# Napoliee/Expressive-FastSpeech2-Mandarin

Hardware: AMD Instinct MI355X
Metric: mel-frames/sec/GPU (batch-64 synth) at 1/2/4/8 MI355X; RTF (higher is better)
Workload: dtype bf16; 1 GPU; cfg2: batch=64 x 64 phonemes per GPU, ESD-Chinese-Singing-MFA model.yaml, FastSpeech2.forward eval bf16; global_batch=64, seq_len=64, mel_frames_per_gpu_batch=24883, T_max=430, parallelism=dp1 (independent shards, no collective), hip_graph=True

## Files before the change

expressive-fastspeech2-mandarin_amd/csrc/ffn_wide.hip:

```cpp
#include <cstdlib>
#include <type_traits>
#include <utility>

#include "conv_common.h"
#include "fs2_common.h"

#ifndef WIDE_TRACE
#define WIDE_TRACE 0
#endif

namespace {

constexpr int kWD = 256;
constexpr int kWUnit = 4096;
constexpr int kWLgkm0 = 0xC07F;

template <int N, typename Fn, int... I>
__device__ __forceinline__ void wfor_impl(Fn &&f, std::integer_sequence<int, I...>) {
  (f(std::integral_constant<int, I>{}), ...);
}
template <int N, typename Fn>
__device__ __forceinline__ void wfor(Fn &&f) {
  wfor_impl<N>(f, std::make_integer_sequence<int, N>{});
}

struct WideArgs {
  const bf16 *x;
  int64_t xs;
  uint32_t x_bytes;
  const bf16 *w;
  uint32_t w_bytes;
  const float *b1, *b2, *gamma, *beta;
  float eps;
  const int64_t *lens;
  const float *av1, *av2;
  const int *rows_dev;
  const int2 *row_pos;
  int M, T, pad, F;
  bf16 *h;
  uint32_t h_bytes;
  int *cnt;
  float *z;
  uint32_t z_bytes;
  bf16 *out;
  int64_t os;
  int nslices, ntiles;
  uint64_t *trace;
};

struct Stamps {
  uint64_t t[8];
  int n = 0;
  __device__ __forceinline__ void at() {
    if (WIDE_TRACE) {
      __builtin_amdgcn_sched_barrier(0);
      t[n++] = __builtin_readcyclecounter();
      __builtin_amdgcn_sched_barrier(0);
    }
  }
  __device__ __forceinline__ void put(uint64_t *tr, int slot) {
    if (WIDE_TRACE && tr != nullptr && threadIdx.x == 0 && slot < 512) {
      for (int i = 0; i < n; ++i) tr[slot * 8 + i] = t[i];
      tr[slot * 8 + 7] = (uint64_t)n;
    }
  }
};

template <int KS>
__global__ __launch_bounds__(256, 2) void ffn_hidden_kernel(WideArgs p) {
  constexpr int BM = 256, XROWS = BM + KS - 1;
  constexpr int NPC = (XROWS + 15) / 16;
  constexpr int CH = 64 + NPC * 1024;
  constexpr int NCH = kWD / 32;
  constexpr int PPW = (NPC + 3) / 4;
  constexpr int NSLOT = 3;
  constexpr int SMEM = NSLOT * CH;
  static_assert(2 * SMEM <= 163840, "two workgroups per CU");
  static_assert(BM * 144 <= SMEM, "H staging fits in the ring");
  static_assert((NSLOT - 1) * CH < 65536, "slot offsets fit the ds_read immediate");
  constexpr int NK = KS * NCH;
  constexpr int MB = 8;
  __shared__ __attribute__((aligned(16))) char smem[SMEM];
  Stamps st;
  st.at();

  const int tid = threadIdx.x, lane = tid & 63;
  const int w = __builtin_amdgcn_readfirstlane(tid >> 6);
  const int rh = w & 1, hh = w >> 1;
  const int L = (blockIdx.x & 7) * (gridDim.x >> 3) + (blockIdx.x >> 3);
  const int slice = L / p.ntiles, tile = L - slice * p.ntiles;
  if (slice >= p.nslices) return;
  const int M = p.rows_dev != nullptr ? min(*p.rows_dev, p.M) : p.M;
  const int m0 = tile * BM;
  if (m0 >= M) return;
  const int pad = p.pad, T = p.T;

  if (tid < NSLOT * 4) *reinterpret_cast<float4 *>(smem + (tid >> 2) * CH + (tid & 3) * 16) = make_float4(0.f, 0.f, 0.f, 0.f);
  int2 rq[MB];
#pragma unroll
  for (int mb = 0; mb < MB; ++mb) {
    const int m = min(m0 + rh * 128 + mb * 16 + (lane & 15), M - 1);
    rq[mb] = make_int2(m % T, T);
  }
  if (p.row_pos != nullptr) {
#pragma unroll
    for (int mb = 0; mb < MB; ++mb) rq[mb] = p.row_pos[min(m0 + rh * 128 + mb * 16 + (lane & 15), M - 1)];
  }
  const int hcol0 = slice * 64 + hh * 32 + 4 * (lane >> 4);
  const float4 bb0 = *reinterpret_cast<const float4 *>(p.b1 + hcol0);
  const float4 bb1 = *reinterpret_cast<const float4 *>(p.b1 + hcol0 + 16);
  const rsrc_t sr = make_rsrc(p.x, p.x_bytes);
  const uint32_t srow = (uint32_t)p.xs * 2u;
  auto dma_chunk = [&](auto CI) {
    constexpr int c = decltype(CI)::value;
    const int ps = lane & 3;
#pragma unroll
    for (int i = 0; i < PPW; ++i) {
      const int pc = min(w + 4 * i, NPC - 1);
      const int R = pc * 16 + (lane >> 2);
      const int hl = ps ^ ((R >> 1) & 2);
      const int gm = m0 - pad + R;
      const bool ok = R < XROWS && gm >= 0 && gm < M;
      __builtin_amdgcn_raw_ptr_buffer_load_lds(
          sr, (__attribute__((address_space(3))) void *)(smem + (c % NSLOT) * CH + 64 + pc * 1024), 16,
          ok ? (uint32_t)gm * srow + (uint32_t)(c * 64 + hl * 16) : kOOB, 0, 0, 0);
    }
  };
  dma_chunk(std::integral_constant<int, 0>{});
  dma_chunk(std::integral_constant<int, 1>{});

  constexpr int RD = 6;
  const rsrc_t wr = make_rsrc(p.w, p.w_bytes);
  const uint32_t wbase = (uint32_t)(slice * NK) * (uint32_t)kWUnit + (uint32_t)(hh * 2048 + lane * 16);
  bf16x8 pa[RD][2];
  auto load_at = [&](auto KI) {
    constexpr int kk = decltype(KI)::value, c = kk / KS, t = kk % KS;
    __builtin_amdgcn_sched_barrier(0);
    const uint32_t o = wbase + (uint32_t)(t * NCH + c) * (uint32_t)kWUnit;
    pa[kk % RD][0] = __builtin_bit_cast(bf16x8, __builtin_amdgcn_raw_buffer_load_b128(wr, o, 0, 0));
    pa[kk % RD][1] = __builtin_bit_cast(bf16x8, __builtin_amdgcn_raw_buffer_load_b128(wr, o + 1024, 0, 0));
    __builtin_amdgcn_sched_barrier(0);
  };
  wfor<RD>([&](auto I) { load_at(I); });
  auto refills = [](int a, int b) constexpr {
    int n = 0;
    for (int kk = a; kk <= b; ++kk) n += kk + RD < NK ? 2 : 0;
    return n;
  };

  const int r16 = lane & 15, hi = lane >> 4;
  uint32_t adp[KS][MB / 2];
  {
    asm volatile("s_waitcnt vmcnt(%0)" ::"n"(2 * PPW + 2 * RD) : "memory");
#pragma unroll
    for (int t = 0; t < KS; ++t) {
      const int R0 = rh * 128 + r16 + t;
      const int sl = (hi ^ ((R0 >> 1) & 2)) * 16;
#pragma unroll
      for (int i = 0; i < MB / 2; ++i) {
        uint32_t a2[2];
#pragma unroll
        for (int j = 0; j < 2; ++j) {
          const int mb = 2 * i + j;
          const bool ok = (unsigned)(rq[mb].x + t - pad) < (unsigned)rq[mb].y;
          a2[j] = ok ? (uint32_t)(64 + (R0 + 16 * mb) * 64 + sl) : 0u;
        }
        adp[t][i] = a2[0] | (a2[1] << 16);
      }
    }
  }
  static_assert(CH < 65536, "16-bit fragment addresses");
  auto wait_chunk = [&](auto CI) {
    constexpr int c = decltype(CI)::value;
    constexpr int n = c == 0 ? PPW + 2 * RD
                             : c == 1 ? 2 * RD + refills(0, KS - 2)
                                      : refills((c - 2) * KS + KS - 1, (c - 1) * KS + KS - 2);
    static_assert(n <= 63, "vmcnt");
    asm volatile("s_waitcnt vmcnt(%0)" ::"n"(n) : "memory");
    __builtin_amdgcn_s_waitcnt(kWLgkm0);
    __builtin_amdgcn_sched_barrier(0);
    __builtin_amdgcn_s_barrier();
    __builtin_amdgcn_sched_barrier(0);
  };
  wait_chunk(std::integral_constant<int, 0>{});
  st.at();

  f32x4 acc[2][MB];
#pragma unroll
  for (int jb = 0; jb < 2; ++jb)
#pragma unroll
    for (int mb = 0; mb < MB; ++mb) acc[jb][mb] = f32x4{0.f, 0.f, 0.f, 0.f};
  auto issue = [&](auto CI, auto TI, bf16x8 (&f)[MB]) {
    constexpr int c = decltype(CI)::value, t = decltype(TI)::value, off = (c % NSLOT) * CH;
#pragma unroll
    for (int mb = 0; mb < MB; ++mb) {
      uint32_t a;
      asm volatile("v_bfe_u32 %0, %1, %2, 16" : "=v"(a) : "v"(adp[t][mb >> 1]), "n"((mb & 1) * 16));
      f[mb] = *reinterpret_cast<const bf16x8 *>(smem + a + off);
    }
  };
  auto mma = [&](const bf16x8 (&fa)[2], const bf16x8 (&fb)[MB]) {
#pragma unroll
    for (int mb = 0; mb < MB; ++mb)
#pragma unroll
      for (int jb = 0; jb < 2; ++jb)
        acc[jb][mb] = __builtin_amdgcn_mfma_f32_16x16x32_bf16(fa[jb], fb[mb], acc[jb][mb], 0, 0, 0);
  };
  bf16x8 f0[MB], f1[MB];
  issue(std::integral_constant<int, 0>{}, std::integral_constant<int, 0>{}, f0);
  wfor<NCH>([&](auto CI) {
    constexpr int c = decltype(CI)::value;
    wfor<KS>([&](auto TI) {
      constexpr int t = decltype(TI)::value;
      constexpr int kk = c * KS + t;
      if constexpr (t + 1 < KS) {
        if constexpr (kk & 1)
          issue(CI, std::integral_constant<int, t + 1>{}, f0);
        else
          issue(CI, std::integral_constant<int, t + 1>{}, f1);
      } else if constexpr (c + 1 < NCH) {
        wait_chunk(std::integral_constant<int, c + 1>{});
        if constexpr (c + 2 < NCH) dma_chunk(std::integral_constant<int, c + 2>{});
        if constexpr (kk & 1)
          issue(std::integral_constant<int, c + 1>{}, std::integral_constant<int, 0>{}, f0);
        else
          issue(std::integral_constant<int, c + 1>{}, std::integral_constant<int, 0>{}, f1);
      }
      if constexpr (kk & 1)
        mma(pa[kk % RD], f1);
      else
        mma(pa[kk % RD], f0);
      if constexpr (kk + RD < NK) load_at(std::integral_constant<int, kk + RD>{});
    });
  });
  __builtin_amdgcn_s_waitcnt(kWLgkm0);
  __builtin_amdgcn_s_barrier();
  st.at();

  constexpr int HP = 144;
  const int hrow0 = rh * 128 + r16;
#pragma unroll
  for (int jb = 0; jb < 2; ++jb) {
    const float4 bb = jb == 0 ? bb0 : bb1;
#pragma unroll
    for (int mb = 0; mb < MB; ++mb) {
      const f32x4 v = acc[jb][mb];
      bf16x4 o;
      o[0] = (bf16)fmaxf(v[0] + bb.x, 0.f);
      o[1] = (bf16)fmaxf(v[1] + bb.y, 0.f);
      o[2] = (bf16)fmaxf(v[2] + bb.z, 0.f);
      o[3] = (bf16)fmaxf(v[3] + bb.w, 0.f);
      *reinterpret_cast<bf16x4 *>(smem + (hrow0 + 16 * mb) * HP + (hh * 32 + jb * 16 + 4 * hi) * 2) = o;
    }
  }
  __builtin_amdgcn_s_waitcnt(kWLgkm0);
  __syncthreads();
  const uint32_t hrow = (uint32_t)p.F * 2u;
  char *hb = reinterpret_cast<char *>(p.h);
#pragma unroll
  for (int i = 0; i < BM * 8 / 256; ++i) {
    const int e = tid + 256 * i, r = e >> 3, c = e & 7;
    if (m0 + r < M)
      *reinterpret_cast<uint4 *>(hb + (uint32_t)(m0 + r) * hrow + (uint32_t)(slice * 128 + c * 16)) =
          *reinterpret_cast<const uint4 *>(smem + r * HP + c * 16);
  }
  if (WIDE_TRACE) {
    asm volatile("s_waitcnt vmcnt(0)" ::: "memory");
    st.at();
    st.put(p.trace, L);
  }
}

__device__ __forceinline__ void ln_row(const WideArgs &p, f32x4 (&v)[16], int m, int hi, const char *vec, char *dst) {
  bool masked = false;
  int bb = 0;
  if (p.row_pos == nullptr) {
    bb = m / p.T;
    masked = p.lens != nullptr && (int64_t)(m - bb * p.T) >= p.lens[bb];
  }
  float4 a1[16], a2[16];
#pragma unroll
  for (int i = 0; i < 16; ++i) {
    const int n = 16 * i + 4 * hi;
    a1[i] = p.av1 != nullptr ? *reinterpret_cast<const float4 *>(p.av1 + (int64_t)bb * kWD + n) : make_float4(0.f, 0.f, 0.f, 0.f);
  }
  float s = 0.f;
#pragma unroll
  for (int i = 0; i < 16; ++i) s += (v[i][0] + v[i][1]) + (v[i][2] + v[i][3]);
  s += __shfl_xor(s, 16, 64);
  s += __shfl_xor(s, 32, 64);
  const float mean = s * (1.0f / 256.0f);
  float ss = 0.f;
#pragma unroll
  for (int i = 0; i < 16; ++i) {
    v[i] -= mean;
    ss += (v[i][0] * v[i][0] + v[i][1] * v[i][1]) + (v[i][2] * v[i][2] + v[i][3] * v[i][3]);
  }
  ss += __shfl_xor(ss, 16, 64);
  ss += __shfl_xor(ss, 32, 64);
  const float rstd = 1.0f / sqrtf(ss * (1.0f / 256.0f) + p.eps);
#pragma unroll
  for (int i = 0; i < 16; ++i) {
    const int n = 16 * i + 4 * hi;
    a2[i] = p.av2 != nullptr ? *reinterpret_cast<const float4 *>(p.av2 + (int64_t)bb * kWD + n) : make_float4(0.f, 0.f, 0.f, 0.f);
  }
  const float *vg = reinterpret_cast<const float *>(vec), *vb = vg + kWD;
#pragma unroll
  for (int i = 0; i < 16; ++i) {
    const int n = 16 * i + 4 * hi;
    const float4 g = *reinterpret_cast<const float4 *>(vg + n);
    const float4 be = *reinterpret_cast<const float4 *>(vb + n);
    float y[4] = {v[i][0] * rstd * g.x + be.x, v[i][1] * rstd * g.y + be.y, v[i][2] * rstd * g.z + be.z,
                  v[i][3] * rstd * g.w + be.w};
    if (masked) y[0] = y[1] = y[2] = y[3] = 0.f;
    if (p.av1 != nullptr) {
      y[0] += a1[i].x; y[1] += a1[i].y; y[2] += a1[i].z; y[3] += a1[i].w;
    }
    if (p.av2 != nullptr) {
      y[0] += a2[i].x; y[1] += a2[i].y; y[2] += a2[i].z; y[3] += a2[i].w;
    }
    const bf16x4 o = {(bf16)y[0], (bf16)y[1], (bf16)y[2], (bf16)y[3]};
    *reinterpret_cast<bf16x4 *>(dst + n * 2) = o;
  }
}

template <int F, int RB>
__global__ __launch_bounds__(256, 1) void ffn_out_rows_kernel(WideArgs p) {
  constexpr int NK = F / 32;
  constexpr int KW = NK / 4;
  constexpr int BM = 16 * RB;
  constexpr int RD = 3;
  static_assert(KW >= RD && (RD - 1) * (16 + RB) <= 63, "ring");
  constexpr int RED = 4 * 16 * RB * 64 * 16;
  constexpr int ZP = kWD * 4 + 64;
  constexpr int ZB = BM * ZP;
  constexpr int OP = kWD * 2 + 16;
  constexpr int VEC = RED;
  static_assert(ZB + BM * OP <= RED, "pre-norm rows + staging fit over the partials");
  static_assert(RED + 2048 <= 163840, "LDS");
  __shared__ __attribute__((aligned(16))) char smem[RED + 2048];
  Stamps st;
  st.at();

  const int tid = threadIdx.x, lane = tid & 63;
  const int w = __builtin_amdgcn_readfirstlane(tid >> 6);
  const int L = (blockIdx.x & 7) * (gridDim.x >> 3) + (blockIdx.x >> 3);
  if (L >= p.ntiles) return;
  const int M = p.rows_dev != nullptr ? min(*p.rows_dev, p.M) : p.M;
  const int m0 = L * BM;
  if (m0 >= M) return;
  const int hi = lane >> 4, r16 = lane & 15;
  if (w < 2)
    __builtin_amdgcn_raw_ptr_buffer_load_lds(make_rsrc(w == 0 ? p.gamma : p.beta, 1024),
                                             (__attribute__((address_space(3))) void *)(smem + VEC + w * 1024), 16,
                                             (uint32_t)lane * 16u, 0, 0, 0);
  const rsrc_t xr = make_rsrc(p.x, p.x_bytes);
  float4 b2v[4];
  uint2 xv[RB][4];
#pragma unroll
  for (int jb = 0; jb < 4; ++jb) {
    const int n = 64 * w + 16 * jb + 4 * hi;
    b2v[jb] = *reinterpret_cast<const float4 *>(p.b2 + n);
#pragma unroll
    for (int mb = 0; mb < RB; ++mb) {
      const int m = m0 + 16 * mb + r16;
      xv[mb][jb] = bload8(xr, m < M ? (uint32_t)m * (uint32_t)p.xs * 2u + (uint32_t)n * 2u : kOOB);
    }
  }

  const rsrc_t wr = make_rsrc(p.w, p.w_bytes);
  const rsrc_t hr = make_rsrc(p.h, p.h_bytes);
  const uint32_t wb = p.w_bytes - (uint32_t)(kWD * F * 2) + (uint32_t)(w * KW * kWUnit) + (uint32_t)lane * 16u;
  const uint32_t hrow = (uint32_t)F * 2u;
  uint32_t hoff[RB];
#pragma unroll
  for (int mb = 0; mb < RB; ++mb) {
    const int m = m0 + 16 * mb + r16;
    hoff[mb] = m < M ? (uint32_t)m * hrow + (uint32_t)(w * KW * 64 + hi * 16) : kOOB;
  }
  bf16x8 wa[RD][16], hb[RD][RB];
  auto load_at = [&](auto KI) {
    constexpr int k = decltype(KI)::value;
    __builtin_amdgcn_sched_barrier(0);
#pragma unroll
    for (int J = 0; J < 16; ++J)
      wa[k % RD][J] = __builtin_bit_cast(
          bf16x8, __builtin_amdgcn_raw_buffer_load_b128(wr, wb + (uint32_t)(((J >> 2) * NK + k) * kWUnit + (J & 3) * 1024), 0, 0));
#pragma unroll
    for (int mb = 0; mb < RB; ++mb)
      hb[k % RD][mb] = __builtin_bit_cast(bf16x8, __builtin_amdgcn_raw_buffer_load_b128(hr, hoff[mb] + (uint32_t)(k * 64), 0, 0));
    __builtin_amdgcn_sched_barrier(0);
  };
  wfor<RD>([&](auto I) { load_at(I); });
  if (WIDE_TRACE) st.at();

  f32x4 acc[16][RB];
#pragma unroll
  for (int J = 0; J < 16; ++J)
#pragma unroll
    for (int mb = 0; mb < RB; ++mb) acc[J][mb] = f32x4{0.f, 0.f, 0.f, 0.f};
  wfor<KW>([&](auto KI) {
    constexpr int k = decltype(KI)::value;
#pragma unroll
    for (int mb = 0; mb < RB; ++mb)
#pragma unroll
      for (int J = 0; J < 16; ++J)
        acc[J][mb] = __builtin_amdgcn_mfma_f32_16x16x32_bf16(wa[k % RD][J], hb[k % RD][mb], acc[J][mb], 0, 0, 0);
    if constexpr (k + RD < KW) load_at(std::integral_constant<int, k + RD>{});
  });
  f32x4 *red = reinterpret_cast<f32x4 *>(smem);
#pragma unroll
  for (int J = 0; J < 16; ++J)
#pragma unroll
    for (int mb = 0; mb < RB; ++mb) red[((w * 16 + J) * RB + mb) * 64 + lane] = acc[J][mb];
  asm volatile("s_waitcnt vmcnt(0)" ::: "memory");
  __builtin_amdgcn_s_waitcnt(kWLgkm0);
  __builtin_amdgcn_s_barrier();
  st.at();
  f32x4 zv[RB][4];
#pragma unroll
  for (int mb = 0; mb < RB; ++mb)
#pragma unroll
    for (int jb = 0; jb < 4; ++jb) {
      const int J = 4 * w + jb;
      f32x4 s = red[((0 * 16 + J) * RB + mb) * 64 + lane];
#pragma unroll
      for (int ww = 1; ww < 4; ++ww) s += red[((ww * 16 + J) * RB + mb) * 64 + lane];
      const bf16x4 x4 = __builtin_bit_cast(bf16x4, xv[mb][jb]);
      s[0] = s[0] + b2v[jb].x + (float)x4[0];
      s[1] = s[1] + b2v[jb].y + (float)x4[1];
      s[2] = s[2] + b2v[jb].z + (float)x4[2];
      s[3] = s[3] + b2v[jb].w + (float)x4[3];
      zv[mb][jb] = s;
    }
  __builtin_amdgcn_s_waitcnt(kWLgkm0);
  __builtin_amdgcn_s_barrier();
#pragma unroll
  for (int mb = 0; mb < RB; ++mb)
#pragma unroll
    for (int jb = 0; jb < 4; ++jb)
      *reinterpret_cast<f32x4 *>(smem + (16 * mb + r16) * ZP + (64 * w + 16 * jb + 4 * hi) * 4) = zv[mb][jb];
  __builtin_amdgcn_s_waitcnt(kWLgkm0);
  __builtin_amdgcn_s_barrier();
  st.at();
  if (w < RB && m0 + 16 * w + r16 < M) {
    f32x4 v[16];
#pragma unroll
    for (int i = 0; i < 16; ++i) v[i] = *reinterpret_cast<const f32x4 *>(smem + (16 * w + r16) * ZP + (16 * i + 4 * hi) * 4);
    ln_row(p, v, m0 + 16 * w + r16, hi, smem + VEC, smem + ZB + (16 * w + r16) * OP);
  }
  __builtin_amdgcn_s_waitcnt(kWLgkm0);
  __builtin_amdgcn_s_barrier();
#pragma unroll
  for (int i = 0; i < BM * 32 / 256; ++i) {
    const int e = tid + 256 * i, r = e >> 5, c = e & 31;
    if (m0 + r < M)
      *reinterpret_cast<uint4 *>(p.out + (int64_t)(m0 + r) * p.os + c * 8) =
          *reinterpret_cast<const uint4 *>(smem + ZB + r * OP + c * 16);
  }
  if (WIDE_TRACE) {
    asm volatile("s_waitcnt vmcnt(0)" ::: "memory");
    st.at();
    st.put(p.trace, L);
  }
}

template <int F>
__global__ __launch_bounds__(256, 1) void ffn_out_kernel(WideArgs p) {
  constexpr int NK = F / 32;
  constexpr int KW = NK / 4;
  constexpr int RED = 4 * 16 * 64 * 16;
  constexpr int VEC = RED;
  constexpr int OP = kWD * 2 + 16;
  static_assert(64 * OP <= RED, "staging fits");
  __shared__ __attribute__((aligned(16))) char smem[RED + 2048 + 16];
  Stamps st;
  st.at();

  const int tid = threadIdx.x, lane = tid & 63;
  const int w = __builtin_amdgcn_readfirstlane(tid >> 6);
  const int L = (blockIdx.x & 7) * (gridDim.x >> 3) + (blockIdx.x >> 3);
  const int tile = L >> 2, q = L & 3;
  if (tile >= p.ntiles) return;
  const int M = p.rows_dev != nullptr ? min(*p.rows_dev, p.M) : p.M;
  const int m0 = tile * 64;
  if (m0 >= M) return;
  const int hi = lane >> 4, r16 = lane & 15;
  if (w < 2)
    __builtin_amdgcn_raw_ptr_buffer_load_lds(make_rsrc(w == 0 ? p.gamma : p.beta, 1024),
                                             (__attribute__((address_space(3))) void *)(smem + VEC + w * 1024), 16,
                                             (uint32_t)lane * 16u, 0, 0, 0);

  const rsrc_t wr = make_rsrc(p.w, p.w_bytes);
  const rsrc_t hr = make_rsrc(p.h, p.h_bytes);
  bf16x8 wa[KW][4], hb[KW][4];
  const uint32_t wb = p.w_bytes - (uint32_t)(kWD * F * 2) + (uint32_t)((q * NK + w * KW) * kWUnit) + (uint32_t)lane * 16u;
  const uint32_t hrow = (uint32_t)F * 2u;
#pragma unroll
  for (int k = 0; k < KW; ++k) {
#pragma unroll
    for (int jb = 0; jb < 4; ++jb)
      wa[k][jb] = __builtin_bit_cast(bf16x8, __builtin_amdgcn_raw_buffer_load_b128(wr, wb + k * kWUnit + jb * 1024, 0, 0));
#pragma unroll
    for (int mb = 0; mb < 4; ++mb) {
      const int m = m0 + mb * 16 + r16;
      hb[k][mb] = __builtin_bit_cast(
          bf16x8, __builtin_amdgcn_raw_buffer_load_b128(
                      hr, m < M ? (uint32_t)m * hrow + (uint32_t)((w * KW + k) * 64 + hi * 16) : kOOB, 0, 0));
    }
  }
  const int m = m0 + 16 * w + r16;
  const bool mok = m < M;
  const rsrc_t xr = make_rsrc(p.x, p.x_bytes);
  const rsrc_t zr = make_rsrc(p.z, p.z_bytes);
  float4 b2v[4];
  uint2 xv[4];
#pragma unroll
  for (int jb = 0; jb < 4; ++jb) {
    const int n = 64 * q + 16 * jb + 4 * hi;
    b2v[jb] = *reinterpret_cast<const float4 *>(p.b2 + n);
    xv[jb] = bload8(xr, mok ? (uint32_t)m * (uint32_t)p.xs * 2u + (uint32_t)n * 2u : kOOB);
  }
  __builtin_amdgcn_sched_barrier(0);
  if (WIDE_TRACE) {
    asm volatile("s_waitcnt vmcnt(0)" ::: "memory");
    st.at();
  }
  f32x4 acc[4][4];
#pragma unroll
  for (int jb = 0; jb < 4; ++jb)
#pragma unroll
    for (int mb = 0; mb < 4; ++mb) acc[jb][mb] = f32x4{0.f, 0.f, 0.f, 0.f};
#pragma unroll
  for (int k = 0; k < KW; ++k)
#pragma unroll
    for (int mb = 0; mb < 4; ++mb)
#pragma unroll
      for (int jb = 0; jb < 4; ++jb)
        acc[jb][mb] = __builtin_amdgcn_mfma_f32_16x16x32_bf16(wa[k][jb], hb[k][mb], acc[jb][mb], 0, 0, 0);
  f32x4 *red = reinterpret_cast<f32x4 *>(smem);
#pragma unroll
  for (int jb = 0; jb < 4; ++jb)
#pragma unroll
    for (int mb = 0; mb < 4; ++mb) red[(w * 16 + jb * 4 + mb) * 64 + lane] = acc[jb][mb];
  __builtin_amdgcn_s_waitcnt(kWLgkm0);
  __builtin_amdgcn_s_barrier();
  st.at();
  f32x4 zv[4];
#pragma unroll
  for (int jb = 0; jb < 4; ++jb) {
    f32x4 s = red[(0 * 16 + jb * 4 + w) * 64 + lane];
#pragma unroll
    for (int ww = 1; ww < 4; ++ww) s += red[(ww * 16 + jb * 4 + w) * 64 + lane];
    zv[jb] = s;
  }
#pragma unroll
  for (int jb = 0; jb < 4; ++jb) {
    const int n = 64 * q + 16 * jb + 4 * hi;
    const bf16x4 x4 = __builtin_bit_cast(bf16x4, xv[jb]);
    f32x4 v = zv[jb];
    v[0] = v[0] + b2v[jb].x + (float)x4[0];
    v[1] = v[1] + b2v[jb].y + (float)x4[1];
    v[2] = v[2] + b2v[jb].z + (float)x4[2];
    v[3] = v[3] + b2v[jb].w + (float)x4[3];
    __builtin_amdgcn_raw_buffer_store_b128(__builtin_bit_cast(__attribute__((ext_vector_type(4))) unsigned, v), zr,
                                           mok ? ((uint32_t)m * kWD + (uint32_t)n) * 4u : kOOB, 0, 16);
  }
  asm volatile("s_waitcnt vmcnt(0)" ::: "memory");
  __syncthreads();
  st.at();
  int *flag = reinterpret_cast<int *>(smem + RED + 2048);
  if (tid == 0) {
    const int old = __hip_atomic_fetch_add(p.cnt + tile, 1, __ATOMIC_RELAXED, __HIP_MEMORY_SCOPE_AGENT);
    const int last = old == 3;
    if (last) __hip_atomic_store(p.cnt + tile, 0, __ATOMIC_RELAXED, __HIP_MEMORY_SCOPE_AGENT);
    *flag = last;
  }
  __syncthreads();
  st.at();
  if (!*flag) {
    st.put(p.trace, L);
    return;
  }

  if (mok) {
    f32x4 v[16];
#pragma unroll
    for (int i = 0; i < 16; ++i)
      v[i] = __builtin_bit_cast(f32x4, __builtin_amdgcn_raw_buffer_load_b128(
                                           zr, ((uint32_t)m * kWD + (uint32_t)(16 * i + 4 * hi)) * 4u, 0, 16));
    ln_row(p, v, m, hi, smem + VEC, smem + (16 * w + r16) * OP);
  }
  __builtin_amdgcn_s_waitcnt(kWLgkm0);
  __builtin_amdgcn_s_barrier();
#pragma unroll
  for (int i = 0; i < 8; ++i) {
    const int e = tid + 256 * i, r = e >> 5, c = e & 31;
    if (m0 + r < M)
      *reinterpret_cast<uint4 *>(p.out + (int64_t)(m0 + r) * p.os + c * 8) =
          *reinterpret_cast<const uint4 *>(smem + r * OP + c * 16);
  }
  if (WIDE_TRACE) {
    asm volatile("s_waitcnt vmcnt(0)" ::: "memory");
    st.at();
    st.put(p.trace, L);
  }
}

}

extern "C" int fs2_ffn_wide(const fs2_ffn_desc *d, void *hidden, int64_t hidden_bytes, fs2_stream_t stream) {
  if (d == nullptr || d->x == nullptr || d->w == nullptr || d->b1 == nullptr || d->b2 == nullptr ||
      d->ln_gamma == nullptr || d->ln_beta == nullptr || d->out == nullptr || hidden == nullptr)
    return FS2_EINVAL;
  if (d->B < 0 || d->T < 0 || d->x_row_stride < kWD || (d->x_row_stride & 7) || d->out_row_stride < kWD ||
      (d->out_row_stride & 7))
    return FS2_EINVAL;
  if (d->D != kWD || !(d->F == 1024 || d->F == 512) || !(d->KS == 9 || d->KS == 3) || d->pad < 0 ||
      d->pad > d->KS - 1)
    return FS2_EUNSUPPORTED;
  if (d->wqkv != nullptr || d->pre_att != nullptr) return FS2_EUNSUPPORTED;
  if ((d->rows_dev == nullptr) != (d->row_pos == nullptr)) return FS2_EINVAL;
  if (d->rows_dev != nullptr && (d->lens != nullptr || d->addvec1 != nullptr || d->addvec2 != nullptr))
    return FS2_EINVAL;
  if (d->x == d->out || hidden == d->x || hidden == d->out) return FS2_EINVAL;
  const int64_t M64 = (int64_t)d->B * d->T;
  if (M64 > 0x7fffff00LL || d->rows_max < 0) return FS2_EINVAL;
  if (M64 == 0) return FS2_OK;
  const int64_t Mg = (d->rows_dev != nullptr && d->rows_max > 0 && d->rows_max < M64) ? d->rows_max : M64;
  const int64_t xb = M64 * d->x_row_stride * 2;
  const int64_t wb = ((int64_t)d->F * d->KS * kWD + (int64_t)kWD * d->F) * 2;
  const int64_t hb = Mg * d->F * 2;
  const int ntiles64 = (int)((Mg + 63) / 64);
  const int64_t zb = Mg * kWD * 4;
  if (xb >= (1LL << 31) || hb >= (1LL << 31) || hidden_bytes < hb) return FS2_EUNSUPPORTED;
  if (d->splitk_ws == nullptr || ntiles64 > 1024 || d->splitk_ws_bytes < 4096 + zb || zb >= (1LL << 31))
    return FS2_EINVAL;
  WideArgs p{};
  p.x = reinterpret_cast<const bf16 *>(d->x);
  p.xs = d->x_row_stride;
  p.x_bytes = (uint32_t)xb;
  p.w = reinterpret_cast<const bf16 *>(d->w);
  p.w_bytes = (uint32_t)wb;
  p.b1 = d->b1;
  p.b2 = d->b2;
  p.gamma = d->ln_gamma;
  p.beta = d->ln_beta;
  p.eps = d->ln_eps;
  p.lens = d->lens;
  p.av1 = d->addvec1;
  p.av2 = d->addvec2;
  p.rows_dev = d->rows_dev;
  p.row_pos = reinterpret_cast<const int2 *>(d->row_pos);
  p.M = (int)Mg;
  p.T = d->T;
  p.pad = d->pad;
  p.F = d->F;
  p.h = static_cast<bf16 *>(hidden);
  p.h_bytes = (uint32_t)hb;
  p.cnt = static_cast<int *>(d->splitk_ws);
  p.z = reinterpret_cast<float *>(static_cast<char *>(d->splitk_ws) + 4096);
  p.z_bytes = (uint32_t)zb;
  p.out = static_cast<bf16 *>(d->out);
  p.os = d->out_row_stride;
  if (WIDE_TRACE)
    p.trace = reinterpret_cast<uint64_t *>(static_cast<char *>(d->splitk_ws) + d->splitk_ws_bytes - 65536);
  hipStream_t s = as_stream(stream);
  p.nslices = d->F / 64;
  p.ntiles = (int)((Mg + 255) / 256);
  const int n1 = (p.nslices * p.ntiles + 7) & ~7;
  constexpr int kCUs = 256;
  constexpr int kRowsRounds = 2;
  const size_t solo = 32 * 1024;
  if (d->KS == 9)
    hipLaunchKernelGGL((ffn_hidden_kernel<9>), dim3(n1), dim3(256), n1 <= kCUs ? solo : 0, s, p);
  else
    hipLaunchKernelGGL((ffn_hidden_kernel<3>), dim3(n1), dim3(256), n1 <= kCUs ? solo : 0, s, p);
  FS2_CHECK_LAUNCH();
  if (WIDE_TRACE) p.trace += 4096;
  {
    const char *e = getenv("FS2_WIDE_OUT"), *f = getenv("FS2_WIDE_OUT_RB");
    int rb = 0;
    if (e == nullptr || e[0] != '0') {
      if (f != nullptr && (f[0] == '1' || f[0] == '2'))
        rb = f[0] - '0';
      else
        rb = Mg <= 16 * kCUs ? 1 : Mg <= 32 * kRowsRounds * kCUs ? 2 : 0;
    }
    if (rb != 0) {
      p.ntiles = (int)((Mg + 16 * rb - 1) / (16 * rb));
      const int nr = (p.ntiles + 7) & ~7;
      if (d->F == 1024 && rb == 1)
        hipLaunchKernelGGL((ffn_out_rows_kernel<1024, 1>), dim3(nr), dim3(256), 0, s, p);
      else if (d->F == 1024)
        hipLaunchKernelGGL((ffn_out_rows_kernel<1024, 2>), dim3(nr), dim3(256), 0, s, p);
      else if (rb == 1)
        hipLaunchKernelGGL((ffn_out_rows_kernel<512, 1>), dim3(nr), dim3(256), 0, s, p);
      else
        hipLaunchKernelGGL((ffn_out_rows_kernel<512, 2>), dim3(nr), dim3(256), 0, s, p);
      FS2_CHECK_LAUNCH();
      return FS2_OK;
    }
  }
  p.ntiles = ntiles64;
  const int n2 = (ntiles64 * 4 + 7) & ~7;
  if (d->F == 1024)
    hipLaunchKernelGGL((ffn_out_kernel<1024>), dim3(n2), dim3(256), 0, s, p);
  else
    hipLaunchKernelGGL((ffn_out_kernel<512>), dim3(n2), dim3(256), 0, s, p);
  FS2_CHECK_LAUNCH();
  return FS2_OK;
}
```

Baseline: 18.17 million mel-frames/s.

## Use 8-wave workgroups for FFN hidden kernel when grid underfills CUs

Templates the FFN hidden conv-GEMM kernel on wave count, so an 8-wave (512-thread) variant splits each 256-row tile into four row groups of 64 rows instead of two of 128. The 8-wave version is picked when the grid is no larger than the CU count, and an env var can force either variant. The aim is more waves per CU for latency hiding and less per-wave work in the underfilled case. In exchange it runs one workgroup per CU, and the trace also records hardware IDs.

```diff
diff --git a/expressive-fastspeech2-mandarin_amd/csrc/ffn_wide.hip b/expressive-fastspeech2-mandarin_amd/csrc/ffn_wide.hip
--- a/expressive-fastspeech2-mandarin_amd/csrc/ffn_wide.hip
+++ b/expressive-fastspeech2-mandarin_amd/csrc/ffn_wide.hip
@@ -61,32 +61,37 @@
   __device__ __forceinline__ void put(uint64_t *tr, int slot) {
     if (WIDE_TRACE && tr != nullptr && threadIdx.x == 0 && slot < 512) {
       for (int i = 0; i < n; ++i) tr[slot * 8 + i] = t[i];
+      tr[slot * 8 + 6] = (uint64_t)__builtin_amdgcn_s_getreg(4 | (31 << 11)) |
+                         ((uint64_t)__builtin_amdgcn_s_getreg(20 | (31 << 11)) << 32);
       tr[slot * 8 + 7] = (uint64_t)n;
     }
   }
 };
 
-template <int KS>
-__global__ __launch_bounds__(256, 2) void ffn_hidden_kernel(WideArgs p) {
+template <int KS, int NW>
+__global__ __launch_bounds__(NW * 64, NW == 8 ? 1 : 2) void ffn_hidden_kernel(WideArgs p) {
+  static_assert(NW == 4 || NW == 8, "waves");
+  constexpr int NT = NW * 64, NRP = NW / 2;
   constexpr int BM = 256, XROWS = BM + KS - 1;
   constexpr int NPC = (XROWS + 15) / 16;
   constexpr int CH = 64 + NPC * 1024;
   constexpr int NCH = kWD / 32;
-  constexpr int PPW = (NPC + 3) / 4;
+  constexpr int PPW = (NPC + NW - 1) / NW;
   constexpr int NSLOT = 3;
   constexpr int SMEM = NSLOT * CH;
   static_assert(2 * SMEM <= 163840, "two workgroups per CU");
   static_assert(BM * 144 <= SMEM, "H staging fits in the ring");
   static_assert((NSLOT - 1) * CH < 65536, "slot offsets fit the ds_read immediate");
   constexpr int NK = KS * NCH;
-  constexpr int MB = 8;
+  constexpr int RH = BM / NRP;
+  constexpr int MB = RH / 16;
   __shared__ __attribute__((aligned(16))) char smem[SMEM];
   Stamps st;
   st.at();
 
   const int tid = threadIdx.x, lane = tid & 63;
   const int w = __builtin_amdgcn_readfirstlane(tid >> 6);
-  const int rh = w & 1, hh = w >> 1;
+  const int rh = w & (NRP - 1), hh = w / NRP;
   const int L = (blockIdx.x & 7) * (gridDim.x >> 3) + (blockIdx.x >> 3);
   const int slice = L / p.ntiles, tile = L - slice * p.ntiles;
   if (slice >= p.nslices) return;
@@ -99,12 +104,12 @@
   int2 rq[MB];
 #pragma unroll
   for (int mb = 0; mb < MB; ++mb) {
-    const int m = min(m0 + rh * 128 + mb * 16 + (lane & 15), M - 1);
+    const int m = min(m0 + rh * RH + mb * 16 + (lane & 15), M - 1);
     rq[mb] = make_int2(m % T, T);
   }
   if (p.row_pos != nullptr) {
 #pragma unroll
-    for (int mb = 0; mb < MB; ++mb) rq[mb] = p.row_pos[min(m0 + rh * 128 + mb * 16 + (lane & 15), M - 1)];
+    for (int mb = 0; mb < MB; ++mb) rq[mb] = p.row_pos[min(m0 + rh * RH + mb * 16 + (lane & 15), M - 1)];
   }
   const int hcol0 = slice * 64 + hh * 32 + 4 * (lane >> 4);
   const float4 bb0 = *reinterpret_cast<const float4 *>(p.b1 + hcol0);
@@ -116,7 +121,7 @@
     const int ps = lane & 3;
 #pragma unroll
     for (int i = 0; i < PPW; ++i) {
-      const int pc = min(w + 4 * i, NPC - 1);
+      const int pc = min(w + NW * i, NPC - 1);
       const int R = pc * 16 + (lane >> 2);
       const int hl = ps ^ ((R >> 1) & 2);
       const int gm = m0 - pad + R;
@@ -154,7 +159,7 @@
     asm volatile("s_waitcnt vmcnt(%0)" ::"n"(2 * PPW + 2 * RD) : "memory");
 #pragma unroll
     for (int t = 0; t < KS; ++t) {
-      const int R0 = rh * 128 + r16 + t;
+      const int R0 = rh * RH + r16 + t;
       const int sl = (hi ^ ((R0 >> 1) & 2)) * 16;
 #pragma unroll
       for (int i = 0; i < MB / 2; ++i) {
@@ -238,7 +243,7 @@
   st.at();
 
   constexpr int HP = 144;
-  const int hrow0 = rh * 128 + r16;
+  const int hrow0 = rh * RH + r16;
 #pragma unroll
   for (int jb = 0; jb < 2; ++jb) {
     const float4 bb = jb == 0 ? bb0 : bb1;
@@ -258,8 +263,8 @@
   const uint32_t hrow = (uint32_t)p.F * 2u;
   char *hb = reinterpret_cast<char *>(p.h);
 #pragma unroll
-  for (int i = 0; i < BM * 8 / 256; ++i) {
-    const int e = tid + 256 * i, r = e >> 3, c = e & 7;
+  for (int i = 0; i < BM * 8 / NT; ++i) {
+    const int e = tid + NT * i, r = e >> 3, c = e & 7;
     if (m0 + r < M)
       *reinterpret_cast<uint4 *>(hb + (uint32_t)(m0 + r) * hrow + (uint32_t)(slice * 128 + c * 16)) =
           *reinterpret_cast<const uint4 *>(smem + r * HP + c * 16);
@@ -671,11 +676,20 @@
   const int n1 = (p.nslices * p.ntiles + 7) & ~7;
   constexpr int kCUs = 256;
   constexpr int kRowsRounds = 2;
-  const size_t solo = 32 * 1024;
-  if (d->KS == 9)
-    hipLaunchKernelGGL((ffn_hidden_kernel<9>), dim3(n1), dim3(256), n1 <= kCUs ? solo : 0, s, p);
+  int nw = n1 <= kCUs ? 8 : 4;
+  {
+    const char *e = getenv("FS2_WIDE_HIDDEN_NW");
+    if (e != nullptr && (e[0] == '4' || e[0] == '8')) nw = e[0] - '0';
+  }
+  const size_t solo = nw == 4 && n1 <= kCUs ? 32 * 1024 : 0;
+  if (d->KS == 9 && nw == 8)
+    hipLaunchKernelGGL((ffn_hidden_kernel<9, 8>), dim3(n1), dim3(512), 0, s, p);
+  else if (d->KS == 9)
+    hipLaunchKernelGGL((ffn_hidden_kernel<9, 4>), dim3(n1), dim3(256), solo, s, p);
+  else if (nw == 8)
+    hipLaunchKernelGGL((ffn_hidden_kernel<3, 8>), dim3(n1), dim3(512), 0, s, p);
   else
-    hipLaunchKernelGGL((ffn_hidden_kernel<3>), dim3(n1), dim3(256), n1 <= kCUs ? solo : 0, s, p);
+    hipLaunchKernelGGL((ffn_hidden_kernel<3, 4>), dim3(n1), dim3(256), solo, s, p);
   FS2_CHECK_LAUNCH();
   if (WIDE_TRACE) p.trace += 4096;
   {
```

Result: slower. 17.98 million mel-frames/s (-1.1%).
